# synsense/HaghighatshoarMuir2024

Measured on AMD Instinct MI355X. Metric: audio samples/sec through STHT+RZCC+SNN beamform, 7-mic 48kHz 360-DoA; DoA MAE vs ref, higher is better.
Workload: dtype f64

## Files before the change

haghighatshoarmuir2024_amd/csrc/beamform_lean.hip:

```cpp
#include "micloc_internal.h"

namespace micloc {

namespace {

typedef double double4_t __attribute__((ext_vector_type(4)));
typedef double double2_t __attribute__((ext_vector_type(2)));
typedef unsigned uint2_t __attribute__((ext_vector_type(2)));

constexpr int LEAN_THREADS = BF_WAVES * 64;
constexpr int LEAN_NT = 2;
constexpr int LEAN_CH = BF_WAVES * LEAN_NT * 16;
constexpr int LEAN_TILES = LEAN_CH / 16;
constexpr int LEAN_C = 14;
constexpr int LEAN_KM = 3, LEAN_KV = 2;

__device__ __forceinline__ void lean_chunk_order(int &chunk, int &b)
{
    const int nchunks = gridDim.x, nb = gridDim.y;
    const int L = chunk + nchunks * b;
    const int full = (nb >> 3) << 3;
    if (L < full * nchunks) {
        const int j = L >> 3;
        const int bq = j / nchunks;
        chunk = j - bq * nchunks;
        b = 8 * bq + (L & 7);
    }
}

__device__ __forceinline__ double lean_row_sum4(double x)
{
    unsigned lo = __double2loint(x), hi = __double2hiint(x);
    uint2_t a = __builtin_amdgcn_permlane16_swap(lo, lo, false, false);
    uint2_t b = __builtin_amdgcn_permlane16_swap(hi, hi, false, false);
    const double s = __hiloint2double(b[0], a[0]) + __hiloint2double(b[1], a[1]);
    lo = __double2loint(s);
    hi = __double2hiint(s);
    a = __builtin_amdgcn_permlane32_swap(lo, lo, false, false);
    b = __builtin_amdgcn_permlane32_swap(hi, hi, false, false);
    return __hiloint2double(b[0], a[0]) + __hiloint2double(b[1], a[1]);
}

__device__ __forceinline__ double lean_row_sum4_pair(double a, double b)
{
    uint2_t lo = __builtin_amdgcn_permlane16_swap(__double2loint(a), __double2loint(b), false, false);
    uint2_t hi = __builtin_amdgcn_permlane16_swap(__double2hiint(a), __double2hiint(b), false, false);
    const double s = __hiloint2double(hi[0], lo[0]) + __hiloint2double(hi[1], lo[1]);
    const unsigned sl = __double2loint(s), sh = __double2hiint(s);
    lo = __builtin_amdgcn_permlane32_swap(sl, sl, false, false);
    hi = __builtin_amdgcn_permlane32_swap(sh, sh, false, false);
    return __hiloint2double(hi[0], lo[0]) + __hiloint2double(hi[1], lo[1]);
}

template <int NG>
__device__ __forceinline__ void lean_stage2(const double *Vl, const double *__restrict__ Wp, int Gp, int wv, int l, int ntile,
                                            double *__restrict__ pout)
{
    const int lc = l & 15;
    const int q = l >> 4;
    double Wf[NG][LEAN_KM], Wv[NG][LEAN_KV];
    const unsigned of = (unsigned)(q * Gp + lc), ov = (unsigned)lc;
#pragma unroll
    for (int j = 0; j < NG; ++j) {
        const double *wp = Wp + 16 * (wv + BF_WAVES * j);
#pragma unroll
        for (int k = 0; k < LEAN_KM; ++k) Wf[j][k] = (wp + (size_t)(4 * k) * Gp)[of];
#pragma unroll
        for (int i = 0; i < LEAN_KV; ++i) Wv[j][i] = (wp + (size_t)(4 * LEAN_KM + i) * Gp)[ov];
    }
    double sq[NG];
#pragma unroll
    for (int j = 0; j < NG; ++j) sq[j] = 0.0;
    const double *pf = Vl + l;
    const double *pt = Vl + 64 * LEAN_KM + q;
    auto tile_step = [&](const int tile) {
        double V[LEAN_KM];
#pragma unroll
        for (int k = 0; k < LEAN_KM; ++k) V[k] = pf[256 * tile + 64 * k];
        double4_t acc[NG];
#pragma unroll
        for (int k = 0; k < LEAN_KM; ++k)
#pragma unroll
            for (int j = 0; j < NG; ++j)
                acc[j] = __builtin_amdgcn_mfma_f64_16x16x4f64(V[k], Wf[j][k], k == 0 ? double4_t{0.0, 0.0, 0.0, 0.0} : acc[j], 0, 0, 0);
#pragma unroll
        for (int i = 0; i < LEAN_KV; ++i) {
            double Vv[4];
#pragma unroll
            for (int r = 0; r < 4; ++r) Vv[r] = pt[256 * tile + 16 * i + 4 * r];
#pragma unroll
            for (int j = 0; j < NG; ++j)
#pragma unroll
                for (int r = 0; r < 4; ++r) acc[j][r] = __builtin_fma(Vv[r], Wv[j][i], acc[j][r]);
        }
#pragma unroll
        for (int r = 0; r < 4; ++r)
#pragma unroll
            for (int j = 0; j < NG; ++j) sq[j] = __builtin_fma(acc[j][r], acc[j][r], sq[j]);
    };
#pragma unroll 1
    for (int t = 0; t < ntile; ++t) tile_step(t);
    if constexpr (NG >= 2) {
        const double s = lean_row_sum4_pair(sq[0], sq[1]);
        if (l < 32) pout[16 * (wv + BF_WAVES * q) + lc] = s;
    } else {
        const double s = lean_row_sum4(sq[0]);
        if (l < 16) pout[16 * wv + l] = s;
    }
    if constexpr (NG == 3) {
        const double s = lean_row_sum4(sq[2]);
        if (l < 16) pout[16 * (wv + BF_WAVES * 2) + l] = s;
    }
}

}

template <int NK, int NGW>
__global__ __launch_bounds__(LEAN_THREADS, 6) void beamform_ws_kernel_lean(const int8_t *__restrict__ spikes, const double *__restrict__ ntab_g,
                                                                            const double *__restrict__ Wp, int GT, int T,
                                                                            double *__restrict__ partial)
{
    constexpr int R = LEAN_CH + 4 * NK - 16;
    constexpr int NTAB = 4 * NK + 16;
    constexpr int NB8 = R * LEAN_C / 8;
    static_assert(R * 16 >= LEAN_TILES * 256, "the parked fragments alias the spike tile");
    static_assert((R * LEAN_C) % 8 == 0 && 4 * NB8 < 13000, "wide staging: whole 8-byte words, and the division by 7 below");
    __shared__ __attribute__((aligned(16))) double smem[R * 16 + NTAB];
    double *S = smem;
    double *Vl = smem;
    double *ntab = smem + R * 16;
    const int Gp = 16 * GT;
    const int tid = threadIdx.x;
    const int wv = __builtin_amdgcn_readfirstlane(tid >> 6);
    const int l = tid & 63;
    const int lc = l & 15;
    const int q = l >> 4;
    int chunk = blockIdx.x, b = blockIdx.y;
    lean_chunk_order(chunk, b);
    const int nchunks = gridDim.x;
    const int cs = chunk * LEAN_CH;

    for (int e = tid; e < NTAB; e += LEAN_THREADS) ntab[e] = ntab_g[e];
    {
        const int8_t *sb = spikes + (size_t)b * T * LEAN_C;
        const int tau0 = cs + 16 - 4 * NK;
        if (tau0 >= 0 && tau0 + R <= T) {
            const int8_t *src = sb + (size_t)tau0 * LEAN_C;
            for (int i = tid; i < NB8; i += LEAN_THREADS) {
                uint2_t w;
                __builtin_memcpy(&w, src + 8 * i, 8);
                const int row0 = (4 * i * 9363) >> 16;
                const int col0 = 8 * i - LEAN_C * row0;
                const int k = (LEAN_C - col0) >> 1;
                double *d = S + row0 * 16 + col0;
#pragma unroll
                for (int p = 0; p < 4; ++p) {
                    const unsigned h = w[p >> 1] >> (16 * (p & 1));
                    double2_t v;
                    v[0] = (double)(int)(int8_t)(h & 0xff);
                    v[1] = (double)(int)(int8_t)((h >> 8) & 0xff);
                    double *dp = (p > 0 && p >= k) ? d + 2 : d;
                    *reinterpret_cast<double2_t *>(dp + 2 * p) = v;
                }
            }
            for (int rho = tid; rho < R; rho += LEAN_THREADS) *reinterpret_cast<double2_t *>(S + rho * 16 + LEAN_C) = double2_t{0.0, 0.0};
        } else {
            const int c = tid & 15;
            constexpr int RP = LEAN_THREADS / 16;
            const int rr = tid >> 4;
            if (c >= LEAN_C) {
                for (int rho = rr; rho < R; rho += RP) S[rho * 16 + c] = 0.0;
            } else {
                for (int r0 = rr; r0 < R; r0 += RP * 6) {
                    int8_t v[6];
#pragma unroll
                    for (int i = 0; i < 6; ++i) {
                        int tau = tau0 + r0 + RP * i;
                        tau = tau < 0 ? 0 : (tau >= T ? T - 1 : tau);
                        v[i] = sb[(size_t)tau * LEAN_C + c];
                    }
#pragma unroll
                    for (int i = 0; i < 6; ++i) {
                        const int rho = r0 + RP * i;
                        const int tau = tau0 + rho;
                        if (rho < R) S[rho * 16 + c] = (tau >= 0 && tau < T) ? (double)v[i] : 0.0;
                    }
                }
            }
        }
    }
    __syncthreads();

    const int tb0 = cs + wv * LEAN_NT * 16;
    const bool active = tb0 < T;
    double4_t vacc[LEAN_NT];
    if (active) {
        const double *sp = S + (wv * LEAN_NT * 16 + q) * 16 + lc;
        const double *np_ = ntab + (lc - q + 3);
#pragma unroll
        for (int ks = 0; ks < NK; ++ks) {
            const double bn = np_[4 * (NK - 1 - ks)];
            double a[LEAN_NT];
#pragma unroll
            for (int tt = 0; tt < LEAN_NT; ++tt) a[tt] = sp[(16 * tt + 4 * ks) * 16];
#pragma unroll
            for (int tt = 0; tt < LEAN_NT; ++tt)
                vacc[tt] = __builtin_amdgcn_mfma_f64_16x16x4f64(a[tt], bn, ks == 0 ? double4_t{0.0, 0.0, 0.0, 0.0} : vacc[tt], 0, 0, 0);
        }
    }
    __syncthreads();
    if (active) {
        if (tb0 + LEAN_NT * 16 > T) {
#pragma unroll
            for (int tt = 0; tt < LEAN_NT; ++tt) {
                const bool tvalid = (tb0 + 16 * tt + lc) < T;
#pragma unroll
                for (int r = 0; r < 4; ++r) vacc[tt][r] = tvalid ? vacc[tt][r] : 0.0;
            }
        }
#pragma unroll
        for (int tt = 0; tt < LEAN_NT; ++tt) {
            double *vp = Vl + (wv * LEAN_NT + tt) * 256 + l;
#pragma unroll
            for (int r = 0; r < 4; ++r) vp[64 * r] = vacc[tt][r];
        }
    }
    __syncthreads();

    int ntile = (T - cs + 15) >> 4;
    ntile = ntile > LEAN_TILES ? LEAN_TILES : ntile;
    double *pout = partial + ((size_t)b * nchunks + chunk) * Gp;
    const bool owns_all = wv + BF_WAVES * (NGW - 1) < GT;
    if (owns_all)
        lean_stage2<NGW>(Vl, Wp, Gp, wv, l, ntile, pout);
    else
        lean_stage2<NGW - 1>(Vl, Wp, Gp, wv, l, ntile, pout);
}

bool launch_lif_beamform_lean(const BeamformW &W, const NeuronTab &nt, const int8_t *spikes, int B, int T, double *y, double *partial,
                              hipStream_t stream, int *nchunks, hipError_t *err)
{
    if (VARIANT_WS_GENERAL_ONLY) return false;
    if (y || !partial || W.chunk_range || W.complex_pairs || W.CT != 1 || W.C != LEAN_C) return false;
    if ((W.GT + BF_WAVES - 1) / BF_WAVES != 3) return false;
    const int nch = (T + LEAN_CH - 1) / LEAN_CH;
    const dim3 grid(nch, B), block(LEAN_THREADS);
    switch (nt.NK) {
        case 13:
            hipLaunchKernelGGL((beamform_ws_kernel_lean<13, 3>), grid, block, 0, stream, spikes, nt.tab, W.Wp, W.GT, T, partial);
            break;
        default: return false;
    }
    *nchunks = nch;
    *err = hipGetLastError();
    return true;
}

}
```

Measured before the change: 3.873 billion.

## Replace MFMA Toeplitz neuron filter with direct FIR on channel-major spike tile

When the neuron kernel has 35 taps, the lean beamform kernel no longer builds a Toeplitz MFMA product from a padded row-major spike tile. It stages spikes channel-major with an odd-pair pitch and has each lane compute eight consecutive outputs with scalar FMAs over a register window, reading taps straight from global memory. This drops the padded Toeplitz work and the neuron-table staging, but moves the filter onto vector FMA units and adds strided LDS stores during staging.

```diff
diff --git a/haghighatshoarmuir2024_amd/csrc/beamform_lean.hip b/haghighatshoarmuir2024_amd/csrc/beamform_lean.hip
--- a/haghighatshoarmuir2024_amd/csrc/beamform_lean.hip
+++ b/haghighatshoarmuir2024_amd/csrc/beamform_lean.hip
@@ -115,20 +115,25 @@
 
 }
 
-template <int NK, int NGW>
+template <int NK, int NGW, int NTAPS>
 __global__ __launch_bounds__(LEAN_THREADS, 6) void beamform_ws_kernel_lean(const int8_t *__restrict__ spikes, const double *__restrict__ ntab_g,
                                                                             const double *__restrict__ Wp, int GT, int T,
                                                                             double *__restrict__ partial)
 {
+    constexpr bool FIR = NTAPS > 0;
     constexpr int R = LEAN_CH + 4 * NK - 16;
-    constexpr int NTAB = 4 * NK + 16;
+    constexpr int FP = R + 2;
+    constexpr int FOFF = 4 * NK - 16 - (NTAPS - 1);
+    constexpr int NTAB = FIR ? 0 : 4 * NK + 16;
+    constexpr int NSPK = FIR ? LEAN_C * FP : R * 16;
     constexpr int NB8 = R * LEAN_C / 8;
-    static_assert(R * 16 >= LEAN_TILES * 256, "the parked fragments alias the spike tile");
+    static_assert(FIR || R * 16 >= LEAN_TILES * 256, "the parked fragments alias the spike tile");
+    static_assert(!FIR || (FOFF >= 0 && FOFF % 2 == 0 && FP % 4 == 2 && (NTAPS + 7) % 2 == 0), "FIR: 16-byte window reads, conflict-free pitch");
     static_assert((R * LEAN_C) % 8 == 0 && 4 * NB8 < 13000, "wide staging: whole 8-byte words, and the division by 7 below");
-    __shared__ __attribute__((aligned(16))) double smem[R * 16 + NTAB];
+    __shared__ __attribute__((aligned(16))) double smem[(NSPK > LEAN_TILES * 256 ? NSPK : LEAN_TILES * 256) + NTAB];
     double *S = smem;
     double *Vl = smem;
-    double *ntab = smem + R * 16;
+    double *ntab = smem + (NSPK > LEAN_TILES * 256 ? NSPK : LEAN_TILES * 256);
     const int Gp = 16 * GT;
     const int tid = threadIdx.x;
     const int wv = __builtin_amdgcn_readfirstlane(tid >> 6);
@@ -140,7 +145,8 @@
     const int nchunks = gridDim.x;
     const int cs = chunk * LEAN_CH;
 
-    for (int e = tid; e < NTAB; e += LEAN_THREADS) ntab[e] = ntab_g[e];
+    if constexpr (!FIR)
+        for (int e = tid; e < NTAB; e += LEAN_THREADS) ntab[e] = ntab_g[e];
     {
         const int8_t *sb = spikes + (size_t)b * T * LEAN_C;
         const int tau0 = cs + 16 - 4 * NK;
@@ -152,24 +158,37 @@
                 const int row0 = (4 * i * 9363) >> 16;
                 const int col0 = 8 * i - LEAN_C * row0;
                 const int k = (LEAN_C - col0) >> 1;
-                double *d = S + row0 * 16 + col0;
-#pragma unroll
-                for (int p = 0; p < 4; ++p) {
-                    const unsigned h = w[p >> 1] >> (16 * (p & 1));
-                    double2_t v;
-                    v[0] = (double)(int)(int8_t)(h & 0xff);
-                    v[1] = (double)(int)(int8_t)((h >> 8) & 0xff);
-                    double *dp = (p > 0 && p >= k) ? d + 2 : d;
-                    *reinterpret_cast<double2_t *>(dp + 2 * p) = v;
+                if constexpr (FIR) {
+                    double *d = S + col0 * FP + row0;
+#pragma unroll
+                    for (int p = 0; p < 4; ++p) {
+                        const unsigned h = w[p >> 1] >> (16 * (p & 1));
+                        double *dp = (p > 0 && p >= k) ? d + (1 - LEAN_C * FP) : d;
+                        dp[(2 * p) * FP] = (double)(int)(int8_t)(h & 0xff);
+                        dp[(2 * p + 1) * FP] = (double)(int)(int8_t)((h >> 8) & 0xff);
+                    }
+                } else {
+                    double *d = S + row0 * 16 + col0;
+#pragma unroll
+                    for (int p = 0; p < 4; ++p) {
+                        const unsigned h = w[p >> 1] >> (16 * (p & 1));
+                        double2_t v;
+                        v[0] = (double)(int)(int8_t)(h & 0xff);
+                        v[1] = (double)(int)(int8_t)((h >> 8) & 0xff);
+                        double *dp = (p > 0 && p >= k) ? d + 2 : d;
+                        *reinterpret_cast<double2_t *>(dp + 2 * p) = v;
+                    }
                 }
             }
-            for (int rho = tid; rho < R; rho += LEAN_THREADS) *reinterpret_cast<double2_t *>(S + rho * 16 + LEAN_C) = double2_t{0.0, 0.0};
+            if constexpr (!FIR)
+                for (int rho = tid; rho < R; rho += LEAN_THREADS) *reinterpret_cast<double2_t *>(S + rho * 16 + LEAN_C) = double2_t{0.0, 0.0};
         } else {
             const int c = tid & 15;
             constexpr int RP = LEAN_THREADS / 16;
             const int rr = tid >> 4;
             if (c >= LEAN_C) {
-                for (int rho = rr; rho < R; rho += RP) S[rho * 16 + c] = 0.0;
+                if constexpr (!FIR)
+                    for (int rho = rr; rho < R; rho += RP) S[rho * 16 + c] = 0.0;
             } else {
                 for (int r0 = rr; r0 < R; r0 += RP * 6) {
                     int8_t v[6];
@@ -183,7 +202,7 @@
                     for (int i = 0; i < 6; ++i) {
                         const int rho = r0 + RP * i;
                         const int tau = tau0 + rho;
-                        if (rho < R) S[rho * 16 + c] = (tau >= 0 && tau < T) ? (double)v[i] : 0.0;
+                        if (rho < R) S[FIR ? c * FP + rho : rho * 16 + c] = (tau >= 0 && tau < T) ? (double)v[i] : 0.0;
                     }
                 }
             }
@@ -193,36 +212,72 @@
 
     const int tb0 = cs + wv * LEAN_NT * 16;
     const bool active = tb0 < T;
-    double4_t vacc[LEAN_NT];
-    if (active) {
-        const double *sp = S + (wv * LEAN_NT * 16 + q) * 16 + lc;
-        const double *np_ = ntab + (lc - q + 3);
-#pragma unroll
-        for (int ks = 0; ks < NK; ++ks) {
-            const double bn = np_[4 * (NK - 1 - ks)];
-            double a[LEAN_NT];
-#pragma unroll
-            for (int tt = 0; tt < LEAN_NT; ++tt) a[tt] = sp[(16 * tt + 4 * ks) * 16];
-#pragma unroll
-            for (int tt = 0; tt < LEAN_NT; ++tt)
-                vacc[tt] = __builtin_amdgcn_mfma_f64_16x16x4f64(a[tt], bn, ks == 0 ? double4_t{0.0, 0.0, 0.0, 0.0} : vacc[tt], 0, 0, 0);
-        }
-    }
-    __syncthreads();
-    if (active) {
-        if (tb0 + LEAN_NT * 16 > T) {
+    if constexpr (FIR) {
+        constexpr int NW = NTAPS + 7;
+        const int fc = l >> 2, fb = l & 3;
+        const bool mine = active && fc < LEAN_C;
+        double facc[8];
+        if (active) __builtin_amdgcn_s_setprio(3);
+        if (mine) {
+            double tap[NTAPS];
+#pragma unroll
+            for (int k = 0; k < NTAPS; ++k) tap[k] = ntab_g[15 + k];
+            const double2_t *sp = reinterpret_cast<const double2_t *>(S + fc * FP + wv * LEAN_NT * 16 + 8 * fb + FOFF);
+            double wnd[NW];
+#pragma unroll
+            for (int m = 0; m < NW / 2; ++m) {
+                const double2_t v = sp[m];
+                wnd[2 * m] = v[0];
+                wnd[2 * m + 1] = v[1];
+            }
+#pragma unroll
+            for (int s = 0; s < NTAPS; ++s)
+#pragma unroll
+                for (int i = 0; i < 8; ++i) facc[i] = __builtin_fma(tap[NTAPS - 1 - s], wnd[s + i], s == 0 ? 0.0 : facc[i]);
+        }
+        if (active) __builtin_amdgcn_s_setprio(0);
+        __syncthreads();
+        if (mine) {
+            if (tb0 + LEAN_NT * 16 > T) {
+#pragma unroll
+                for (int i = 0; i < 8; ++i) facc[i] = (tb0 + 8 * fb + i) < T ? facc[i] : 0.0;
+            }
+            double2_t *vp = reinterpret_cast<double2_t *>(Vl + (wv * LEAN_NT + (fb >> 1)) * 256 + 16 * fc + 8 * (fb & 1));
+#pragma unroll
+            for (int i = 0; i < 4; ++i) vp[i] = double2_t{facc[2 * i], facc[2 * i + 1]};
+        }
+    } else {
+        double4_t vacc[LEAN_NT];
+        if (active) {
+            const double *sp = S + (wv * LEAN_NT * 16 + q) * 16 + lc;
+            const double *np_ = ntab + (lc - q + 3);
+#pragma unroll
+            for (int ks = 0; ks < NK; ++ks) {
+                const double bn = np_[4 * (NK - 1 - ks)];
+                double a[LEAN_NT];
+#pragma unroll
+                for (int tt = 0; tt < LEAN_NT; ++tt) a[tt] = sp[(16 * tt + 4 * ks) * 16];
+#pragma unroll
+                for (int tt = 0; tt < LEAN_NT; ++tt)
+                    vacc[tt] = __builtin_amdgcn_mfma_f64_16x16x4f64(a[tt], bn, ks == 0 ? double4_t{0.0, 0.0, 0.0, 0.0} : vacc[tt], 0, 0, 0);
+            }
+        }
+        __syncthreads();
+        if (active) {
+            if (tb0 + LEAN_NT * 16 > T) {
+#pragma unroll
+                for (int tt = 0; tt < LEAN_NT; ++tt) {
+                    const bool tvalid = (tb0 + 16 * tt + lc) < T;
+#pragma unroll
+                    for (int r = 0; r < 4; ++r) vacc[tt][r] = tvalid ? vacc[tt][r] : 0.0;
+                }
+            }
 #pragma unroll
             for (int tt = 0; tt < LEAN_NT; ++tt) {
-                const bool tvalid = (tb0 + 16 * tt + lc) < T;
-#pragma unroll
-                for (int r = 0; r < 4; ++r) vacc[tt][r] = tvalid ? vacc[tt][r] : 0.0;
-            }
-        }
-#pragma unroll
-        for (int tt = 0; tt < LEAN_NT; ++tt) {
-            double *vp = Vl + (wv * LEAN_NT + tt) * 256 + l;
-#pragma unroll
-            for (int r = 0; r < 4; ++r) vp[64 * r] = vacc[tt][r];
+                double *vp = Vl + (wv * LEAN_NT + tt) * 256 + l;
+#pragma unroll
+                for (int r = 0; r < 4; ++r) vp[64 * r] = vacc[tt][r];
+            }
         }
     }
     __syncthreads();
@@ -247,7 +302,10 @@
     const dim3 grid(nch, B), block(LEAN_THREADS);
     switch (nt.NK) {
         case 13:
-            hipLaunchKernelGGL((beamform_ws_kernel_lean<13, 3>), grid, block, 0, stream, spikes, nt.tab, W.Wp, W.GT, T, partial);
+            if (nt.n == 35)
+                hipLaunchKernelGGL((beamform_ws_kernel_lean<13, 3, 35>), grid, block, 0, stream, spikes, nt.tab, W.Wp, W.GT, T, partial);
+            else
+                hipLaunchKernelGGL((beamform_ws_kernel_lean<13, 3, 0>), grid, block, 0, stream, spikes, nt.tab, W.Wp, W.GT, T, partial);
             break;
         default: return false;
     }
```

Result: faster. 3.958 billion, median of 6 (+2.2%).
